# Audio-WestlakeU/FN-SSL

Measured on AMD Instinct MI355X. Metric: TF-frames/sec DP-IPD forward, 4-mic 257-bin x 300-frame, higher is better.
Workload: dtype f32; 1 GPU; BASELINE configs[1]: FN-SSL (online) DP-IPD forward, waveform->STFT->features->3x(full-band BiLSTM + narrow-band LSTM)->head; 32 utterances/GPU x 4 mics ('MM' = 6 pairs) x 257 bins x 300 frames, fp32; frame = one STFT frame of one utterance; stream_chunk_frames=0, utterances_per_gpu=32, global_batch=32, mics=4, pairs_per_utterance=6, frames=300, bins=257, parallelism=dp1 (utterance shards, no collective), chunk_pairs=0

## Files before the change

### fn-ssl_amd/csrc/lstm_f32c.h

```cpp
#pragma once

#include "lstm_static.h"

namespace fnssl_lstm {

constexpr int kF32cWaves = 16;

struct F32ClusterParams {
  unsigned* tags;
  unsigned* status;
  int clusters_per_dir;
  int groups_per_cluster;
  unsigned spin_limit;
  int stall_member;
  int rotate;
  int prio_mode;
};

template <int HH, int NV0, int NS0, int MODE, bool ABLRT = false, int DRIFT = 2, int NW_ = kF32cWaves, int GS = 1>
__global__ void __launch_bounds__(NW_ * 64) lstm_f32c_kernel(const LstmParams p, const F32ClusterParams cp) {
  constexpr int H = HH, NS = H / 16, NW = NW_;
  constexpr int NWS = NW / GS;
  static_assert((GS == 1 || GS == 4) && NW % GS == 0 && (NWS & (NWS - 1)) == 0, "gate split: whole slots, a power of two of them");
  constexpr bool SUM = (MODE & kSum) != 0, SAVE = (MODE & kSave) != 0;
  constexpr bool CAT = (MODE & kHas2) != 0;
  constexpr int QPS = 1 + NV0 + NS0 + NS;
  constexpr int XD = NW_ > 12 ? 4 : 8;
  constexpr bool STRH = H == 256 && GS == 1 && NW_ > 8;
  static_assert((CAT ? NS0 == 1 : !(NV0 && NS0)) && (NV0 == 0 || NV0 % XD == 0) && (H == 128 || H == 256),
                "blocks of src0, or its remainder alone, or blocks of src0 + the remainder quad of src2");
  static_assert(H == 128 || NW_ <= 8 || STRH, "H = 256 with the row of h_{t-1} held: at most two waves per SIMD (register budget)");
  static_assert(!STRH || (NV0 >= XD && (NV0 + NS) % XD == 0), "streamed row: the ring depth divides the block count");
  static_assert(GS == 1 || (!SAVE && !ABLRT), "gate split: inference kernels only");
  extern __shared__ __attribute__((aligned(16))) char smem[];
  const int ABL = ABLRT ? p.ablate : 0;

  const int b = blockIdx.x;
  const int m = (b >> 3) % NS;
  const int cl = ((b >> 3) / NS) * 8 + (b & 7);
  if (cl >= cp.clusters_per_dir * p.ndir) return;
  const int dir = cl / cp.clusters_per_dir;
  const int ck = cl - dir * cp.clusters_per_dir;
  const int g0 = ck * cp.groups_per_cluster;
  const int g1 = g0 + cp.groups_per_cluster < p.ntasks ? g0 + cp.groups_per_cluster : p.ntasks;
  if (__hip_atomic_load(cp.status, __ATOMIC_RELAXED, __HIP_MEMORY_SCOPE_AGENT) != 0) return;
  if (cl == 0 && m == cp.stall_member) return;

  const int lane = threadIdx.x & 63;
  const int n = lane & 15, g = lane >> 4;
  const int w = __builtin_amdgcn_readfirstlane((int)(threadIdx.x >> 6));
  const int ws = GS == 1 ? w : (w >> 2);
  const int gate = GS == 1 ? 0 : (w & 3);
  const bool rev = dir == 1;
  const unsigned vlane = lane * 16;

  {
    const v4f* src = reinterpret_cast<const v4f*>(reinterpret_cast<const char*>(p.wpack[dir]) + (size_t)(m * QPS) * 4096);
    v4f* dst = reinterpret_cast<v4f*>(smem);
    for (int i = threadIdx.x; i < QPS * 4 * 64; i += NW * 64) dst[i] = src[i];
  }
  char* const xch = smem + QPS * 4096;
  unsigned* const xcnt = reinterpret_cast<unsigned*>(xch + NWS * 2 * 4 * 1024);
  if (GS > 1 && threadIdx.x < NWS) xcnt[threadIdx.x] = 0;
  __syncthreads();
  const char* const lds_rd = smem + lane * 16;
  auto rec = [&](int q, int j) { return *reinterpret_cast<const v4f*>(lds_rd + (q * 4 + j) * 1024); };
  auto rec1 = [&](int q, int j) { return *reinterpret_cast<const float*>(lds_rd + (q * 4 + j) * 1024 + 4 * gate); };

  const unsigned st0 = (unsigned)(p.src0.st * 4), sto = (unsigned)(p.out_st * 4), stk = SUM ? (unsigned)(p.skip.st * 4) : 0u;
  const unsigned st2 = CAT ? (unsigned)(p.src2.st * 4) : 0u;
  const unsigned cy = (unsigned)p.carry;
  unsigned* const tag_cl = cp.tags + (size_t)cl * cp.groups_per_cluster * NS;
  const v4f zero4 = v4f{0.f, 0.f, 0.f, 0.f};

  unsigned pub_val = 0;
  unsigned* pub_tag = nullptr;
  auto pub_flush = [&]() {
    if (pub_tag) {
      asm volatile("s_waitcnt vmcnt(0)" ::: "memory");
      if (lane == 0) __hip_atomic_store(pub_tag, pub_val, __ATOMIC_RELAXED, __HIP_MEMORY_SCOPE_AGENT);
      pub_tag = nullptr;
    }
  };

  struct Grp {
    unsigned vo0, voo, vok, voo2, vo2 = 0;
    bool valid;
    int task, step;
  };
  auto locate = [&](int task, int qo0, int qi0, Grp& gr, rsrc_t& rx0, rsrc_t& ro, rsrc_t& rsk, rsrc_t& ro2, rsrc_t& rx2) {
    const int q0 = task * 16;
    gr.valid = q0 + n < p.nseq;
    const int d = q0 + n < p.nseq ? n : p.nseq - 1 - q0;
    const bool crossed = qi0 + d >= p.q_inner;
    auto one = [&](const float* base, long long so, long long si, int extra, unsigned& voff) {
      const long long delta = (long long)d * si + (crossed ? so - (long long)p.q_inner * si : 0ll);
      voff = (unsigned)(delta * 4) + (unsigned)(extra * 4);
      return make_rsrc(base + ((long long)qo0 * so + (long long)qi0 * si));
    };
    rx0 = one(p.src0.p, p.src0.so, p.src0.si, (NS0 && !CAT) ? g : 4 * g, gr.vo0);
    if constexpr (CAT) rx2 = one(p.src2.p, p.src2.so, p.src2.si, g, gr.vo2);
    ro = one(p.out, p.out_so, p.out_si, dir * H + 4 * g, gr.voo);
    gr.vok = gr.voo2 = 0;
    rsk = SUM ? one(p.skip.p, p.skip.so, p.skip.si, dir * H + 4 * g, gr.vok) : rx0;
    ro2 = SUM ? one(p.out_sum, p.out_so, p.out_si, dir * H + 4 * g, gr.voo2) : ro;
// ... 3 lines not shown
    return make_rsrc(cell_record<NS>(p.cscratch, p.ntasks, dir, task));
  };

  if (g0 + ws >= g1) return;
  unsigned long long clk0 = 0, rt0 = 0;
  if (ABLRT && (ABL & 512)) {
    clk0 = __builtin_amdgcn_s_memtime();
    rt0 = __builtin_amdgcn_s_memrealtime();
  }
  bool dead = false;
  auto bounded_wait = [&](auto ready, auto reload, int sleep, unsigned code) {
    for (unsigned spins = 0; !ready(); ++spins) {
      if (GS > 1) __builtin_amdgcn_s_sleep(1); else if (sleep == 8) __builtin_amdgcn_s_sleep(8); else __builtin_amdgcn_s_sleep(16);
      reload();
      const bool out = spins > cp.spin_limit;
      if (out || (spins & 63) == 63) {
        if (out) {
          if (lane == 0) __hip_atomic_store(cp.status, code | (unsigned)(cl & 0xffff), __ATOMIC_RELAXED, __HIP_MEMORY_SCOPE_AGENT);
          return false;
        }
        if (__hip_atomic_load(cp.status, __ATOMIC_RELAXED, __HIP_MEMORY_SCOPE_AGENT) != 0) return false;
      }
    }
    return true;
  };
  const int NGR = g1 - g0;
  const bool rot = cp.rotate && NGR >= 2 * NWS;
  const int FULL = rot ? (NGR / NWS) * NWS : NGR, LEFT = NGR - FULL;
  const bool single = GS == 1 && g0 + ws + NWS >= g1;
  Grp cur, nxt;
  rsrc_t rx0, ro, rsk, ro2, rx2, nrx0, nro, nrsk, nro2, nrx2;
  v4f xr[XD];
  float xs0 = 0.f;
  v4f cprev = zero4, skipv = zero4;
  unsigned tagv = 0, tagd = 0;
  auto request = [&](const Grp& gr, rsrc_t qx0, rsrc_t qsk, bool with_c, bool with_x = true) {
    const unsigned tt = tt_of(gr.step);
    if (!(ABL & 8)) {
      if constexpr (NV0 > 0) if (with_x) static_for<XD>([&](auto v) { xr[v.value] = bld4(qx0, gr.vo0, tt * st0 + 64 * v.value); });
      if constexpr (NS0 > 0 && !CAT) xs0 = bld1(qx0, gr.vo0, tt * st0);
    }
    if (SUM && !(ABL & 64)) skipv = bld4(qsk, gr.vok, tt * stk + 64 * m);
    if (gr.step > 0 || cy) {
      if (gr.step > 0 && !(ABL & 256))
        tagv = __hip_atomic_load(tag_cl + (size_t)(gr.task - g0) * NS + (lane & (NS - 1)), __ATOMIC_RELAXED, __HIP_MEMORY_SCOPE_AGENT);
      if (GS == 1 && with_c && !(ABL & 64)) cprev = bld4_l2(rc_of(gr.task), vlane, m * 1024);
    }
    if (DRIFT > 0 && !(ABL & 256) && gr.task - DRIFT * NWS >= g0)
      tagd = __hip_atomic_load(tag_cl + (size_t)(gr.task - DRIFT * NWS - g0) * NS + (lane & (NS - 1)), __ATOMIC_RELAXED, __HIP_MEMORY_SCOPE_AGENT);
  };
  cur.task = g0 + ws;
  cur.step = 0;
  unsigned iter = 0;
  const int qo_first = (cur.task * 16) / p.q_inner, qi_first = cur.task * 16 - qo_first * p.q_inner;
  int qo0 = qo_first, qi0 = qi_first;
  locate(cur.task, qo0, qi0, cur, rx0, ro, rsk, ro2, rx2);
  request(cur, rx0, rsk, true);
  if constexpr (CAT) xs0 = bld1(rx2, cur.vo2, tt_of(0) * st2);

  for (;;) {
    const int step = cur.step, task = cur.task;
    const unsigned tt = tt_of(step);
    const unsigned o0 = tt * st0, oo = (tt + cy) * sto;
    const unsigned op = (rev ? tt + 1 : tt - 1 + cy) * sto;
    const rsrc_t rc = rc_of(task);
    unsigned* const tag_g = tag_cl + (size_t)(task - g0) * NS;
    if (single && (step > 0 || cy) && !(ABL & 64)) cprev = bld4_l2(rc, vlane, m * 1024);
    const bool late_c = GS > 1 || task >= g0 + FULL;
    v4f cprev_cur = (step > 0 || cy) ? cprev : zero4;
    const v4f skip_cur = skipv;

    v4f hold[STRH ? 1 : NS];
    auto fetch_h = [&]() {
      if (DRIFT > 0 && !(ABL & 4) && !dead && task - DRIFT * NWS >= g0) {
        unsigned* const tag_d = tag_cl + (size_t)(task - DRIFT * NWS - g0) * NS;
        dead = !bounded_wait([&]() { return __builtin_amdgcn_ballot_w64(tagd < (unsigned)step + 1) == 0; },
                             [&]() { tagd = __hip_atomic_load(tag_d + (lane & (NS - 1)), __ATOMIC_RELAXED, __HIP_MEMORY_SCOPE_AGENT); }, 8, 0x40000u);
      }
      if ((step > 0 || cy) && !(ABL & 16)) {
        if (step > 0 && !(ABL & 4) && !dead)
          dead = !bounded_wait([&]() { return __builtin_amdgcn_ballot_w64(tagv < (unsigned)step) == 0; },
                               [&]() { tagv = __hip_atomic_load(tag_g + (lane & (NS - 1)), __ATOMIC_RELAXED, __HIP_MEMORY_SCOPE_AGENT); }, 16, 0x30000u);
        if (late_c && !(ABL & 64)) cprev_cur = bld4_l2(rc, vlane, m * 1024);
        if constexpr (!STRH) {
#pragma unroll
          for (int s = 0; s < NS; ++s) hold[s] = bld4_l2(ro, cur.voo, op + 64 * s);
        }
      } else if constexpr (!STRH) {
#pragma unroll
        for (int s = 0; s < NS; ++s) hold[s] = (ABL & 16) ? cprev : zero4;
      }
    };
    const bool hrow = step > 0 || cy;
    auto hblock = [&](int j) { return hrow ? bld4_l2(ro, cur.voo, op + 64 * j) : zero4; };

    if (cp.prio_mode == 2) __builtin_amdgcn_s_setprio(2);
    v4f acc[4];
    v4f ra[4];
    v4f acc1 = zero4;
    float rb[4] = {0.f, 0.f, 0.f, 0.f};
    if constexpr (GS == 1) {
      acc[0] = rec(0, 0);
      acc[1] = rec(0, 1);
      acc[2] = rec(0, 2);
      acc[3] = rec(0, 3);
      static_for<4>([&](auto j) { ra[j.value] = rec(1, j.value); });
    } else {
      acc1 = rec(0, gate);
      static_for<4>([&](auto j) { rb[j.value] = rec1(1, j.value); });
    }
    auto quad = [&](auto qc, float b0, float b1, float b2, float b3) {
      constexpr int Q = decltype(qc)::value;
      if constexpr (GS > 1) {
        acc1 = __builtin_amdgcn_mfma_f32_16x16x4f32(rb[0], b0, acc1, 0, 0, 0);
        if constexpr (Q + 1 < QPS) rb[0] = rec1(Q + 1, 0);
        acc1 = __builtin_amdgcn_mfma_f32_16x16x4f32(rb[1], b1, acc1, 0, 0, 0);
        if constexpr (Q + 1 < QPS) rb[1] = rec1(Q + 1, 1);
        acc1 = __builtin_amdgcn_mfma_f32_16x16x4f32(rb[2], b2, acc1, 0, 0, 0);
        if constexpr (Q + 1 < QPS) rb[2] = rec1(Q + 1, 2);
        acc1 = __builtin_amdgcn_mfma_f32_16x16x4f32(rb[3], b3, acc1, 0, 0, 0);
        if constexpr (Q + 1 < QPS) rb[3] = rec1(Q + 1, 3);
        return;
      }
      MFMA4(acc, ra[0], b0);
      __builtin_amdgcn_sched_barrier(0);
      if constexpr (Q + 1 < QPS) if (!(ABL & 128)) ra[0] = rec(Q + 1, 0);
      __builtin_amdgcn_sched_barrier(0);
      MFMA4(acc, ra[1], b1);
      __builtin_amdgcn_sched_barrier(0);
      if constexpr (Q + 1 < QPS) if (!(ABL & 128)) ra[1] = rec(Q + 1, 1);
      __builtin_amdgcn_sched_barrier(0);
      MFMA4(acc, ra[2], b2);
      __builtin_amdgcn_sched_barrier(0);
      if constexpr (Q + 1 < QPS) if (!(ABL & 128)) ra[2] = rec(Q + 1, 2);
      __builtin_amdgcn_sched_barrier(0);
      MFMA4(acc, ra[3], b3);
      __builtin_amdgcn_sched_barrier(0);
      if constexpr (Q + 1 < QPS) if (!(ABL & 128)) ra[3] = rec(Q + 1, 3);
      __builtin_amdgcn_sched_barrier(0);
    };
    auto quad1 = [&](auto qc, float b0) {
      constexpr int Q = decltype(qc)::value;
      if constexpr (GS > 1) {
        acc1 = __builtin_amdgcn_mfma_f32_16x16x4f32(rb[0], b0, acc1, 0, 0, 0);
        if constexpr (Q + 1 < QPS) static_for<4>([&](auto j) { rb[j.value] = rec1(Q + 1, j.value); });
        return;
      }
      MFMA4(acc, ra[0], b0);
      if constexpr (Q + 1 < QPS) static_for<4>([&](auto j) { ra[j.value] = rec(Q + 1, j.value); });
    };
    if constexpr (NV0 > 0) {
      static_for<NV0>([&](auto v) {
        constexpr int V = decltype(v)::value;
        if constexpr (STRH) {
          if constexpr (V == NV0 / 2) pub_flush();
          if constexpr (V == NV0 - XD) fetch_h();
        } else if constexpr (V == NV0 / 2) {
          pub_flush();
          fetch_h();
        }
        const v4f xb = xr[V % XD];
        quad(ic<1 + V>{}, xb.x, xb.y, xb.z, xb.w);
        if constexpr (V + XD < NV0) {
          if (!(ABL & 8)) xr[V % XD] = bld4(rx0, cur.vo0, o0 + 64 * (V + XD));
        } else if constexpr (STRH) {
          xr[V % XD] = hblock(V + XD - NV0);
        }
      });
      if constexpr (NS0 > 0) quad1(ic<1 + NV0>{}, xs0);
    } else {
      pub_flush();
      fetch_h();
      quad1(ic<1>{}, xs0);
    }
    bool seq_next = false;
    if (task < g0 + FULL && task + NWS < g0 + FULL) {
      nxt.task = task + NWS;
      nxt.step = step;
      seq_next = true;
    } else {
      const int j = (ws - step) & (NWS - 1);
      if (task < g0 + FULL && j < LEFT) {
// ... 20 lines not shown
            qi0 -= p.q_inner;
            ++qo0;
          }
        } else if (nxt.step == step) {
          qo0 = (nxt.task * 16) / p.q_inner;
          qi0 = nxt.task * 16 - qo0 * p.q_inner;
        } else {
          qo0 = qo_first;
          qi0 = qi_first;
        }
        locate(nxt.task, qo0, qi0, nxt, nrx0, nro, nrsk, nro2, nrx2);
      }
      request(nxt, nrx0, nrsk, !single && nxt.task < g0 + FULL, !STRH);
      if constexpr (CAT) xs0 = bld1(nrx2, nxt.vo2, tt_of(nxt.step) * st2);
    }
    static_for<NS>([&](auto sp) {
      constexpr int SP = decltype(sp)::value;
      if constexpr (STRH) {
        constexpr int B = NV0 + SP, B2 = B + XD;
        const v4f hb = xr[B % XD];
        quad(ic<1 + NV0 + NS0 + SP>{}, hb.x, hb.y, hb.z, hb.w);
        if constexpr (B2 < NV0 + NS) {
          xr[B % XD] = hblock(B2 - NV0);
        } else {
          if (more) xr[B % XD] = bld4(nrx0, nxt.vo0, tt_of(nxt.step) * st0 + 64 * (B2 - NV0 - NS));
        }
      } else {
        quad(ic<1 + NV0 + NS0 + SP>{}, hold[SP].x, hold[SP].y, hold[SP].z, hold[SP].w);
      }
    });

    if (cp.prio_mode == 2) __builtin_amdgcn_s_setprio(0);
    if (dead) break;
    v4f cn, hn;
    if (ABL & 2) {
      cn = acc[1] + cprev_cur + acc[0];
      hn = acc[3] + acc[2];
    } else {
      v4f ig, fg, gg, og;
      if constexpr (GS == 1) {
        ig = sigmoid4(acc[0]);
        fg = sigmoid4(acc[1]);
        gg = tanh4(acc[2]);
        og = sigmoid4(acc[3]);
      } else {
        const v4f act = gate == 2 ? tanh4(acc1) : sigmoid4(acc1);
        v4f* const xb = reinterpret_cast<v4f*>(xch + (size_t)((ws * 2 + (int)(iter & 1u)) * 4) * 1024);
        xb[gate * 64 + lane] = act;
        asm volatile("s_waitcnt lgkmcnt(0)" ::: "memory");
        if (lane == 0) __hip_atomic_fetch_add(xcnt + ws, 1u, __ATOMIC_RELAXED, __HIP_MEMORY_SCOPE_WORKGROUP);
        const unsigned want = 4u * (iter + 1u);
        for (unsigned spins = 0;; ++spins) {
          if (__hip_atomic_load(xcnt + ws, __ATOMIC_RELAXED, __HIP_MEMORY_SCOPE_WORKGROUP) >= want) break;
          if (dead || ((spins & 63u) == 63u && __hip_atomic_load(cp.status, __ATOMIC_RELAXED, __HIP_MEMORY_SCOPE_AGENT) != 0u) ||
              spins > cp.spin_limit) {
            dead = true;
            break;
          }
          __builtin_amdgcn_s_sleep(1);
        }
        asm volatile("" ::: "memory");
        ig = xb[lane];
        fg = xb[64 + lane];
        gg = xb[128 + lane];
        og = xb[192 + lane];
        ++iter;
      }
      cn = cell4(fg, cprev_cur, ig, gg);
      hn = mul_rn4(og, tanh4(cn));
      if constexpr (SAVE) {
        const rsrc_t rres = make_rsrc(reinterpret_cast<const char*>(p.reserve) +
                                      ((size_t)dir * p.ntasks + task) * p.nsteps * (size_t)(NS * kReserveRecs * 1024));
        const unsigned rb = (tt * NS + m) * (kReserveRecs * 1024);
        bst4(ig, rres, vlane, rb);
        bst4(fg, rres, vlane, rb + 1024);
        bst4(gg, rres, vlane, rb + 2048);
        bst4(og, rres, vlane, rb + 3072);
        bst4(cn, rres, vlane, rb + 4096);
      }
    }
    asm("" : "+v"(hn.x), "+v"(hn.y), "+v"(hn.z), "+v"(hn.w));
    if (ABL & 32) asm volatile("" ::"v"(cn), "v"(hn));
    const bool storer = GS == 1 || gate == 0;
    if (storer && !(ABL & 32)) bst4(cn, rc, vlane, m * 1024);
    if (storer && cur.valid && !(ABL & 32)) {
      __builtin_amdgcn_raw_buffer_store_b128(__builtin_bit_cast(v4u, hn), ro, cur.voo, oo + 64 * m, 16);
      if (SUM) bst4(add_rn4(hn, skip_cur), ro2, cur.voo2, oo + 64 * m);
    }
    pub_val = __builtin_amdgcn_readfirstlane((unsigned)step + 1);
    pub_tag = ((ABL & 256) || !storer) ? nullptr : tag_g + m;
    if (GS > 1 || single) pub_flush();
    if (!more || dead) break;
    cur = nxt;
    rx0 = nrx0;
    ro = nro;
    rsk = nrsk;
    ro2 = nro2;
    if constexpr (CAT) rx2 = nrx2;
  }
  pub_flush();
  asm volatile("s_waitcnt vmcnt(0)" ::: "memory");
  if (ABLRT && (ABL & 512) && (w == 0 || w == 15) && lane == 0) {
    const unsigned long long c1 = __builtin_amdgcn_s_memtime(), r1 = __builtin_amdgcn_s_memrealtime();
    printf("f32c blk %d wave %d start %llu end %llu cycles %llu MHz %.1f\n", b, w, rt0, r1, c1 - clk0,
           (double)(c1 - clk0) / (double)(r1 - rt0) * 100.0);
  }
}

template <int HH, int NV0, int NS0, int MODE, bool ABLRT = false, int DRIFT = 2, int NW_ = kF32cWaves, int GS = 1>
int launch_f32c_k(const LstmParams& p, const F32ClusterParams& cp, hipStream_t st) {
  constexpr int NS = HH / 16;
  constexpr int QPS = 1 + NV0 + NS0 + NS;
  const size_t lds = (size_t)QPS * 4096 + (GS > 1 ? (size_t)(NW_ / GS) * 8192 + 64 : 0);
  static_assert(QPS * 4096 + (GS > 1 ? (NW_ / GS) * 8192 + 64 : 0) <= 160 * 1024, "LDS");
  auto k = lstm_f32c_kernel<HH, NV0, NS0, MODE, ABLRT, DRIFT, NW_, GS>;
  if (lds > 48 * 1024)
    FNSSL_HIP(hipFuncSetAttribute(reinterpret_cast<const void*>(k), hipFuncAttributeMaxDynamicSharedMemorySize, (int)lds));
  const int ncl = cp.clusters_per_dir * p.ndir;
  const int nwg = 8 * NS * ((ncl + 7) / 8);
  if (!cluster_grid_fits(reinterpret_cast<const void*>(k), NW_ * 64, lds, nwg)) return kNoCluster;
  if (p.dry) return FNSSL_OK;
  hipLaunchKernelGGL(k, dim3(nwg), dim3(NW_ * 64), lds, st, p, cp);
  FNSSL_CHECK_LAUNCH("lstm_f32c_kernel");
  return FNSSL_OK;
}

}
```

### fn-ssl_amd/csrc/lstm_f32c.hip

```cpp
#include <cstdlib>

#include "lstm_f32c.h"
#include "tuning.h"

namespace fnssl_lstm {

constexpr int kF32cWavesH256 = 16;
constexpr int kF32cWavesH256Split = 8;

static bool f32c_uniform(const LstmParams& p, int mode) {
  auto even = [&](long long so, long long si) { return si >= 0 && so == (long long)p.q_inner * si; };
  return even(p.src0.so, p.src0.si) && even(p.out_so, p.out_si) && (!(mode & kSum) || even(p.skip.so, p.skip.si)) &&
         (!(mode & kHas2) || even(p.src2.so, p.src2.si));
}

bool f32c_handles(const LstmParams& p, int H, int mode) {
  if (fnssl::tune(FNSSL_TUNE_NO_F32_CLUSTER)) return false;
  if ((H != 128 && H != 256) || p.ablate) return false;
  if (H == 128) {
    if (p.c2 != 0 || p.carry) return false;
    if (p.reserve && mode != 0) return false;
    if (!(p.c0 == 256 && (mode == kSum || mode == 0)) && !(p.c0 == 4 && mode == 0 && !fnssl::tune(FNSSL_TUNE_NO_F32C_B1))) return false;
  } else {
    if (p.ndir != 1 || p.c0 != 256 || fnssl::tune(FNSSL_TUNE_NO_F32_SMALL)) return false;
    const bool plain = p.c2 == 0 && (mode == 0 || mode == kSum), cat = p.c2 == 4 && (mode == kHas2 || mode == (kHas2 | kSum));
    if (!plain && !cat) return false;
    if (p.reserve && ((mode & kSum) || p.carry)) return false;
  }
  auto grows = [&](long long so, long long si) { return si >= 0 && so >= (long long)(p.q_inner - 1) * si; };
  if (!f32c_uniform(p, mode) &&
      (p.q_inner < 16 || !grows(p.src0.so, p.src0.si) || !grows(p.out_so, p.out_si) ||
       ((mode & kSum) && !grows(p.skip.so, p.skip.si)) || ((mode & kHas2) && !grows(p.src2.so, p.src2.si))))
    return false;
  const int ncu = cluster_cus();
  if (ncu < (H / 16) * p.ndir) return false;
  const long long groups = (long long)p.ntasks * p.ndir;
  if (const int mg = fnssl::tune(FNSSL_TUNE_F32C_MIN_GROUPS, 1, 1 << 30)) {
    if (groups < mg) return false;
  }
  if (p.reserve) {
    if (fnssl::tune(FNSSL_TUNE_TRAIN_NO_F32_CLUSTER)) return false;
    return true;
  }
  if (H == 256) {
    const long long full = 12LL * ncu, rounds = (groups + full - 1) / full;
    return groups < full || groups * 100 < rounds * full * 97;
  }
  return !fnssl::tune(FNSSL_TUNE_NO_F32_SMALL) || groups >= 12LL * ncu;
}

int forward_f32c(LstmParams p, int H, int mode, size_t cluster_bytes, hipStream_t st) {
  if (f32c_uniform(p, mode)) p.q_inner = p.nseq;
  const int ncu = cluster_cus();
  const int members = H / 16;
  F32ClusterParams cp;
  cp.clusters_per_dir = (ncu / members) / p.ndir;
  cp.groups_per_cluster = (p.ntasks + cp.clusters_per_dir - 1) / cp.clusters_per_dir;
  cp.status = reinterpret_cast<unsigned*>(p.cluster_ws);
  cp.tags = reinterpret_cast<unsigned*>(p.cluster_ws + 256);
  cp.spin_limit = cluster_spin_limit();
  cp.stall_member = cluster_test_stall();
  cp.rotate = !fnssl::tune(FNSSL_TUNE_F32C_NO_ROTATE);
  cp.prio_mode = fnssl::tune(FNSSL_TUNE_F32C_PRIO, 9, 9) ? 0 : 2;
  const size_t tag_bytes = (size_t)p.ndir * cp.clusters_per_dir * cp.groups_per_cluster * members * sizeof(unsigned);
  FNSSL_REQUIRE(256 + tag_bytes <= cluster_bytes, "lstm_forward: the cluster kernel's tags exceed the workspace's cluster area");
  if (!p.dry) FNSSL_HIP(hipMemsetAsync(p.cluster_ws, 0, 256 + tag_bytes, st));
  const int gs_knob = fnssl::tune(FNSSL_TUNE_F32C_GATE_SPLIT, 1, 4);
  const bool gsplit = gs_knob ? gs_knob == 4 : cp.groups_per_cluster <= 1;
  if (H == 256) {
    constexpr int W = kF32cWavesH256;
    if (p.reserve)
      return p.c2 == 4 ? launch_f32c_k<256, 16, 1, kHas2 | kSave, false, 2, W>(p, cp, st) : launch_f32c_k<256, 16, 0, kSave, false, 2, W>(p, cp, st);
    if (gsplit) {
      if (mode == (kHas2 | kSum)) return launch_f32c_k<256, 16, 1, kHas2 | kSum, false, 2, kF32cWavesH256Split, 4>(p, cp, st);
      if (mode == kHas2) return launch_f32c_k<256, 16, 1, kHas2, false, 2, kF32cWavesH256Split, 4>(p, cp, st);
      if (mode == kSum) return launch_f32c_k<256, 16, 0, kSum, false, 2, kF32cWavesH256Split, 4>(p, cp, st);
      return launch_f32c_k<256, 16, 0, 0, false, 2, kF32cWavesH256Split, 4>(p, cp, st);
    }
    if (cp.groups_per_cluster <= kF32cWavesH256Split) {
      constexpr int W8 = kF32cWavesH256Split;
      if (mode == (kHas2 | kSum)) return launch_f32c_k<256, 16, 1, kHas2 | kSum, false, 2, W8>(p, cp, st);
      if (mode == kHas2) return launch_f32c_k<256, 16, 1, kHas2, false, 2, W8>(p, cp, st);
      if (mode == kSum) return launch_f32c_k<256, 16, 0, kSum, false, 2, W8>(p, cp, st);
      return launch_f32c_k<256, 16, 0, 0, false, 2, W8>(p, cp, st);
    }
    if (mode == (kHas2 | kSum)) return launch_f32c_k<256, 16, 1, kHas2 | kSum, false, 2, W>(p, cp, st);
    if (mode == kHas2) return launch_f32c_k<256, 16, 1, kHas2, false, 2, W>(p, cp, st);
    if (mode == kSum) return launch_f32c_k<256, 16, 0, kSum, false, 2, W>(p, cp, st);
    return launch_f32c_k<256, 16, 0, 0, false, 2, W>(p, cp, st);
  }
  if (gsplit && !p.reserve) {
    if (p.c0 == 4) return launch_f32c_k<128, 0, 1, 0, false, 2, kF32cWaves, 4>(p, cp, st);
    if (mode == kSum) return launch_f32c_k<128, 16, 0, kSum, false, 2, kF32cWaves, 4>(p, cp, st);
    return launch_f32c_k<128, 16, 0, 0, false, 2, kF32cWaves, 4>(p, cp, st);
  }
#ifdef FNSSL_BUILD_ABLATE
  if (const int abl = env_int("FNSSL_F32C_ABL", 1, 1023)) {
    p.ablate = abl;
    if (mode == kSum) return launch_f32c_k<128, 16, 0, kSum, true>(p, cp, st);
// ... 12 lines not shown
```

### fn-ssl_amd/csrc/runtime.hip

```cpp
#include <atomic>
#include <cstring>
#include <map>
#include <mutex>
#include <string>
#include <vector>

#include "common.h"
#include "tuning.h"

namespace fnssl {

int device_cus() {
  static std::mutex mu;
  static int cache[64] = {0};
  int dev = 0;
  if (hipGetDevice(&dev) != hipSuccess || dev < 0 || dev >= 64) return 256;
  std::lock_guard<std::mutex> lk(mu);
  if (cache[dev] == 0) {
    int n = 0;
    if (hipDeviceGetAttribute(&n, hipDeviceAttributeMultiprocessorCount, dev) != hipSuccess || n <= 0) n = 256;
    cache[dev] = n;
  }
  return cache[dev];
}
// ... 20 lines not shown
    "LSTM_CHQ",
    "NO_F32_CLUSTER",
    "NO_F32C_B1",
    "TRAIN_NO_F32_CLUSTER",
    "F32C_NO_ROTATE",
    "F32C_PRIO",
    "NO_CLUSTER",
    "NO_CLUSTER_B1",
    "NO_CLUSTER_H128",
    "CLUSTER_SPREAD",
    "BF16P_DRAIN",
    "BF16W_SOLO",
    "BWD_NO_CLUSTER",
    "BWD_CLUSTER_MIN_GROUPS",
    "BWD_CLUSTER_NO_ROTATE",
    "BWDC_NO_PREFETCH",
    "BWDC_NO_TOKEN",
    "BWDC_WAVES16",
    "FWD_RING",
    "BWD_RING",
    "TRAIN_SPLIT",
    "TRAIN_NO_STATIC",
    "NO_FWD2",
    "NO_BWD2",
    "SN_SCALAR",
    "STFT_PER_FRAME",
    "CLUSTER_SPIN_LIMIT",
    "CLUSTER_TEST_STALL",
    "RESERVED_CUS",
    "NO_F32_SMALL",
    "F32C_MIN_GROUPS",
    "F32C_GATE_SPLIT",
    "CLUSTER_FULL_TILES",
    "NO_STATIC4"};
constexpr int kTuneNamed = (int)(sizeof(kTuneNames) / sizeof(kTuneNames[0]));
static_assert(kTuneNamed <= FNSSL_TUNE_COUNT, "more knob names than slots");
static_assert(kTuneNamed == FNSSL_TUNE_NO_STATIC4 + 1, "knob names out of step with include/fnssl.h");
}

const fnssl_tuning& tuning() {
  if (g_call_tuning) return *g_call_tuning;
  const unsigned v = g_tuning_version.load(std::memory_order_acquire);
  if (v != g_thread_version) {
    std::lock_guard<std::mutex> lk(g_tuning_mu);
    g_thread_tuning = g_default_tuning;
    g_thread_version = g_tuning_version.load(std::memory_order_relaxed);
  }
  return g_thread_tuning;
}

TuningScope::TuningScope(const fnssl_tuning* t) : prev_(g_call_tuning), active_(false) {
  if (t && t->struct_bytes == sizeof(fnssl_tuning)) {
    g_call_tuning = t;
    active_ = true;
  }
}
TuningScope::~TuningScope() {
  if (active_) g_call_tuning = prev_;
}

void set_error(const char* fmt, ...) {
  va_list ap;
  va_start(ap, fmt);
  vsnprintf(g_err, sizeof(g_err), fmt, ap);
  va_end(ap);
}

namespace {
struct Rec {
  const char* name;
// ... 191 lines not shown
```

### fn-ssl_amd/fnssl/_lib.py

```python
from __future__ import annotations

import ctypes as C
import os

import torch

_HERE = os.path.dirname(os.path.abspath(__file__))
LIB_PATH = os.path.join(os.path.dirname(_HERE), "csrc", "libfnssl_hip.so")
LIB_PATH = os.environ.get("FNSSL_LIB_PATH", LIB_PATH)

ABI_VERSION = 19
CH_MODE = {"M": 0, "MM": 1}
LSTM_FAMILY = {1: "generic", 2: "static", 3: "static2 (retired)", 4: "split", 5: "split_static", 6: "f32_cluster",
               7: "static3", 8: "bf16", 9: "bf16_solo", 10: "bf16_pair", 11: "bf16_cluster", 12: "train", 13: "bwd", 14: "bwd_cluster",
               15: "static4"}

SYMBOLS = [
    "fnssl_abi_version", "fnssl_last_error", "fnssl_tuning_set", "fnssl_tuning_get", "fnssl_tuning_name", "fnssl_occupy_cus", "fnssl_num_frames", "fnssl_num_pairs", "fnssl_stft",
    "fnssl_num_frames_ex", "fnssl_stft_ex", "fnssl_array_frontend",
    "fnssl_forgetting_coefs", "fnssl_pair_features", "fnssl_nchw_to_seq", "fnssl_lstm_packed_floats",
    "fnssl_lstm_pack", "fnssl_lstm_workspace_bytes", "fnssl_lstm_workspace_bytes_ex", "fnssl_lstm_plan_rounds", "fnssl_lstm_plan", "fnssl_lstm_forward", "fnssl_lstm_cluster_status", "fnssl_head", "fnssl_linear",
    "fnssl_ipd2doa", "fnssl_doa_peaks", "fnssl_dpipd_targets", "fnssl_conv3x3_packed_floats", "fnssl_conv3x3_pack", "fnssl_conv3x3_causal",
    "fnssl_avgpool_time", "fnssl_array_features", "fnssl_conv3x3_packed_floats_bf16", "fnssl_conv3x3_pack_bf16",
    "fnssl_conv3x3_causal_bf16", "fnssl_conv3x3_causal_bf16a",
# ... 239 lines not shown
    lib.fnssl_train_map_bytes.restype = sz
    lib.fnssl_train_upload_maps.argtypes = [vp, vp, vp]
    lib.fnssl_train_workspace_bytes.argtypes = [vp, i, i, i]
    lib.fnssl_train_workspace_bytes.restype = sz
    lib.fnssl_train_backward.argtypes = [vp, vp, vp, vp, vp, i, i, i, i, C.c_uint, ll, ll, vp, vp, sz, vp]
    lib.fnssl_train_step.argtypes = [vp, vp, vp, vp, vp, vp, vp, i, i, i, i, C.c_uint, f, f, f, f, i, vp, vp, sz, vp]
    PV = C.POINTER(BtfView)
    lib.fnssl_sn_layernorm.argtypes = [vp, ll, i, vp, vp, f, vp, vp]
    lib.fnssl_sn_encoder.argtypes = [vp, ll, ll, ll, ll, i, i, i, i, vp, vp, vp, vp, vp, ll, ll, ll, i, vp]
    lib.fnssl_sn_fconv.argtypes = [PV, i, i, i, C.POINTER(SnFconvW), i, i, vp, ll, ll, ll, i, vp]
    lib.fnssl_sn_full.argtypes = [PV, i, i, i, C.POINTER(SnFullW), i, vp, ll, ll, ll, i, vp]
    lib.fnssl_sn_mamba_workspace_bytes.argtypes = [i, i, i]
    lib.fnssl_sn_mamba_workspace_bytes.restype = sz
    lib.fnssl_sn_mamba.argtypes = [PV, i, i, i, C.POINTER(SnMambaW), i, i, vp, vp, i, vp, ll, ll, ll, vp, sz, i, vp]
    lib.fnssl_sn_head.argtypes = [PV, i, i, i, vp, vp, vp, vp, vp, vp]
    lib.fnssl_sn_forward_workspace_bytes.argtypes = [i, i, i]
    lib.fnssl_sn_forward_workspace_bytes.restype = sz
    lib.fnssl_sn_state_floats.argtypes = [C.POINTER(SnNet), i, i]
    lib.fnssl_sn_state_floats.restype = sz
    lib.fnssl_sn_forward.argtypes = [C.POINTER(SnNet), vp, ll, ll, ll, ll, i, i, i, vp, i, vp, vp, sz, vp]
    lib.fnssl_timing_enable.argtypes = [i]
    lib.fnssl_timing_select.argtypes = [C.c_char_p]
    lib.fnssl_timing_collect.argtypes = [i, vp, vp, vp, vp]
    if lib.fnssl_abi_version() != ABI_VERSION:
        raise RuntimeError("fnssl: ABI version mismatch (library %d, binding %d)"
                           % (lib.fnssl_abi_version(), ABI_VERSION))
    _lib = lib
    refresh_tuning()
    return lib


_tune_index = None
_PRESENCE = {"NO_F32_CLUSTER", "NO_F32C_B1", "TRAIN_NO_F32_CLUSTER", "F32C_NO_ROTATE", "NO_CLUSTER", "NO_CLUSTER_B1",
             "NO_CLUSTER_H128", "CLUSTER_SPREAD", "BF16W_SOLO", "SN_SCALAR", "STFT_PER_FRAME"}
_ENV_ALIAS = {"LSTM_NO_STATIC": "FNSSL_LSTM_NO_STATIC"}


def tuning_names():
    global _tune_index
    if _tune_index is None:
        lib = _lib
        if lib is None:
            raise RuntimeError("fnssl: load() first")
        idx, k = {}, 0
        while True:
            n = lib.fnssl_tuning_name(k)
            if n is None:
                break
            idx[n.decode()] = k
            k += 1
        _tune_index = idx
    return _tune_index


def tuning_from_env(environ=None) -> Tuning:
    environ = os.environ if environ is None else environ
    t = Tuning()
    t.struct_bytes = C.sizeof(Tuning)
    for name, k in tuning_names().items():
        v = environ.get(_ENV_ALIAS.get(name, "FNSSL_" + name))
        if v is None:
            continue
        try:
            iv = int(v)
        except ValueError:
            iv = 1
        if name in _PRESENCE:
# ... 54 lines not shown
```

### include/fnssl.h

```cpp
#ifndef FNSSL_H_
#define FNSSL_H_

#include <stddef.h>

#ifdef __cplusplus
extern "C" {
#endif

#define FNSSL_ABI_VERSION 19

#define FNSSL_OK 0
#define FNSSL_E_INVALID (-1)
#define FNSSL_E_HIP (-2)
#define FNSSL_E_WORKSPACE (-3)

#define FNSSL_CH_MODE_M 0
#define FNSSL_CH_MODE_MM 1

#define FNSSL_WIN_LEN 512
#define FNSSL_HOP 256
#define FNSSL_NBIN 257
#define FNSSL_NF 256
#define FNSSL_SEG_FRAMES 12

// ... 13 lines not shown
#define FNSSL_TUNE_NO_F32_CLUSTER 9
#define FNSSL_TUNE_NO_F32C_B1 10
#define FNSSL_TUNE_TRAIN_NO_F32_CLUSTER 11
#define FNSSL_TUNE_F32C_NO_ROTATE 12
#define FNSSL_TUNE_F32C_PRIO 13
#define FNSSL_TUNE_NO_CLUSTER 14
#define FNSSL_TUNE_NO_CLUSTER_B1 15
#define FNSSL_TUNE_NO_CLUSTER_H128 16
#define FNSSL_TUNE_CLUSTER_SPREAD 17
#define FNSSL_TUNE_BF16P_DRAIN 18
#define FNSSL_TUNE_BF16W_SOLO 19
#define FNSSL_TUNE_BWD_NO_CLUSTER 20
#define FNSSL_TUNE_BWD_CLUSTER_MIN_GROUPS 21
#define FNSSL_TUNE_BWD_CLUSTER_NO_ROTATE 22
#define FNSSL_TUNE_BWDC_NO_PREFETCH 23
#define FNSSL_TUNE_BWDC_NO_TOKEN 24
#define FNSSL_TUNE_BWDC_WAVES16 25
#define FNSSL_TUNE_FWD_RING 26
#define FNSSL_TUNE_BWD_RING 27
#define FNSSL_TUNE_TRAIN_SPLIT 28
#define FNSSL_TUNE_TRAIN_NO_STATIC 29
#define FNSSL_TUNE_NO_FWD2 30
#define FNSSL_TUNE_NO_BWD2 31
#define FNSSL_TUNE_SN_SCALAR 32
#define FNSSL_TUNE_STFT_PER_FRAME 33
#define FNSSL_TUNE_CLUSTER_SPIN_LIMIT 34
#define FNSSL_TUNE_CLUSTER_TEST_STALL 35
#define FNSSL_TUNE_RESERVED_CUS 36
#define FNSSL_TUNE_NO_F32_SMALL 37
#define FNSSL_TUNE_F32C_MIN_GROUPS 38
#define FNSSL_TUNE_F32C_GATE_SPLIT 39
#define FNSSL_TUNE_CLUSTER_FULL_TILES 40
#define FNSSL_TUNE_NO_STATIC4 41
#define FNSSL_TUNE_COUNT 48

typedef struct fnssl_tuning {
  unsigned struct_bytes;
  int knob[FNSSL_TUNE_COUNT];
} fnssl_tuning;

int fnssl_tuning_set(const fnssl_tuning* t);
int fnssl_tuning_get(fnssl_tuning* t);
const char* fnssl_tuning_name(int index);

int fnssl_occupy_cus(int nblocks, int lds_bytes, unsigned* stop, int max_ms, void* stream);


int fnssl_num_frames(int ns);

int fnssl_num_pairs(int nch, int ch_mode);

int fnssl_stft(const float* sig, int nb, int ns, int nch,
               long long sb, long long sn, long long sc,
               float* spec, float* magsum, void* stream);

int fnssl_num_frames_ex(int ns, int hop, int center);
int fnssl_stft_ex(const float* sig, int nb, int ns, int nch,
                  long long sb, long long sn, long long sc, int hop, int center,
                  float* spec, float* magsum, void* stream);

int fnssl_forgetting_coefs(int nt, int sample_length, float* a, float* b);

int fnssl_pair_features(const float* spec, const float* magsum,
                        const float* coef_a, const float* coef_b,
                        int nb, int nch, int nt, int ch_mode, float eps,
                        float* mu, float* x, int layout, void* stream);
// ... 362 lines not shown
```

Baseline: 17690 frames/s.

## Give each f32 cluster member two hidden slices for block 1 full-band layer

Adds an SPM template parameter so that each cluster workgroup owns two 16-wide hidden slices instead of one. For the H=128 full-band inference layer (c0==4, no reserve), the cluster shrinks from 8 members to 4, which doubles the number of clusters and spreads recurrent groups over more clusters when enough groups exist. Each member now holds twice the weight records in LDS and runs interleaved MFMA chains for both slices. In exchange, per-step work per member doubles and LDS and register use rise, while cross-member tag synchronisation per step drops. A new tuning knob can disable the path.

Result: no change. 17770 frames/s, median of 6 (+0.5%).

```diff
diff --git a/fn-ssl_amd/csrc/lstm_f32c.h b/fn-ssl_amd/csrc/lstm_f32c.h
--- a/fn-ssl_amd/csrc/lstm_f32c.h
+++ b/fn-ssl_amd/csrc/lstm_f32c.h
@@ -17,9 +17,12 @@
   int prio_mode;
 };
 
-template <int HH, int NV0, int NS0, int MODE, bool ABLRT = false, int DRIFT = 2, int NW_ = kF32cWaves, int GS = 1>
+template <int HH, int NV0, int NS0, int MODE, bool ABLRT = false, int DRIFT = 2, int NW_ = kF32cWaves, int GS = 1, int SPM = 1>
 __global__ void __launch_bounds__(NW_ * 64) lstm_f32c_kernel(const LstmParams p, const F32ClusterParams cp) {
   constexpr int H = HH, NS = H / 16, NW = NW_;
+  constexpr int NM = NS / SPM;
+  static_assert(SPM == 1 || (SPM == 2 && H == 128 && NV0 == 0 && NS0 == 1 && MODE == 0 && GS == 1 && !ABLRT),
+                "two slices per member: block 1's full-band inference layer only");
   constexpr int NWS = NW / GS;
   static_assert((GS == 1 || GS == 4) && NW % GS == 0 && (NWS & (NWS - 1)) == 0, "gate split: whole slots, a power of two of them");
   constexpr bool SUM = (MODE & kSum) != 0, SAVE = (MODE & kSave) != 0;
@@ -36,8 +39,8 @@
   const int ABL = ABLRT ? p.ablate : 0;
 
   const int b = blockIdx.x;
-  const int m = (b >> 3) % NS;
-  const int cl = ((b >> 3) / NS) * 8 + (b & 7);
+  const int m = (b >> 3) % NM;
+  const int cl = ((b >> 3) / NM) * 8 + (b & 7);
   if (cl >= cp.clusters_per_dir * p.ndir) return;
   const int dir = cl / cp.clusters_per_dir;
   const int ck = cl - dir * cp.clusters_per_dir;
@@ -55,22 +58,24 @@
   const unsigned vlane = lane * 16;
 
   {
-    const v4f* src = reinterpret_cast<const v4f*>(reinterpret_cast<const char*>(p.wpack[dir]) + (size_t)(m * QPS) * 4096);
+    const v4f* src = reinterpret_cast<const v4f*>(reinterpret_cast<const char*>(p.wpack[dir]) + (size_t)(m * SPM * QPS) * 4096);
     v4f* dst = reinterpret_cast<v4f*>(smem);
-    for (int i = threadIdx.x; i < QPS * 4 * 64; i += NW * 64) dst[i] = src[i];
+    for (int i = threadIdx.x; i < SPM * QPS * 4 * 64; i += NW * 64) dst[i] = src[i];
   }
-  char* const xch = smem + QPS * 4096;
+  char* const xch = smem + SPM * QPS * 4096;
   unsigned* const xcnt = reinterpret_cast<unsigned*>(xch + NWS * 2 * 4 * 1024);
   if (GS > 1 && threadIdx.x < NWS) xcnt[threadIdx.x] = 0;
   __syncthreads();
   const char* const lds_rd = smem + lane * 16;
-  auto rec = [&](int q, int j) { return *reinterpret_cast<const v4f*>(lds_rd + (q * 4 + j) * 1024); };
+  auto recs = [&](int k, int q, int j) { return *reinterpret_cast<const v4f*>(lds_rd + ((k * QPS + q) * 4 + j) * 1024); };
+  auto rec = [&](int q, int j) { return recs(0, q, j); };
   auto rec1 = [&](int q, int j) { return *reinterpret_cast<const float*>(lds_rd + (q * 4 + j) * 1024 + 4 * gate); };
 
   const unsigned st0 = (unsigned)(p.src0.st * 4), sto = (unsigned)(p.out_st * 4), stk = SUM ? (unsigned)(p.skip.st * 4) : 0u;
   const unsigned st2 = CAT ? (unsigned)(p.src2.st * 4) : 0u;
   const unsigned cy = (unsigned)p.carry;
-  unsigned* const tag_cl = cp.tags + (size_t)cl * cp.groups_per_cluster * NS;
+  unsigned* const tag_cl = cp.tags + (size_t)cl * cp.groups_per_cluster * NM;
+  const int s0 = m * SPM;
   const v4f zero4 = v4f{0.f, 0.f, 0.f, 0.f};
 
   unsigned pub_val = 0;
@@ -140,7 +145,8 @@
   rsrc_t rx0, ro, rsk, ro2, rx2, nrx0, nro, nrsk, nro2, nrx2;
   v4f xr[XD];
   float xs0 = 0.f;
-  v4f cprev = zero4, skipv = zero4;
+  v4f cprev[SPM], skipv = zero4;
+  static_for<SPM>([&](auto k) { cprev[k.value] = zero4; });
   unsigned tagv = 0, tagd = 0;
   auto request = [&](const Grp& gr, rsrc_t qx0, rsrc_t qsk, bool with_c, bool with_x = true) {
     const unsigned tt = tt_of(gr.step);
@@ -148,14 +154,15 @@
       if constexpr (NV0 > 0) if (with_x) static_for<XD>([&](auto v) { xr[v.value] = bld4(qx0, gr.vo0, tt * st0 + 64 * v.value); });
       if constexpr (NS0 > 0 && !CAT) xs0 = bld1(qx0, gr.vo0, tt * st0);
     }
-    if (SUM && !(ABL & 64)) skipv = bld4(qsk, gr.vok, tt * stk + 64 * m);
+    if (SUM && !(ABL & 64)) skipv = bld4(qsk, gr.vok, tt * stk + 64 * s0);
     if (gr.step > 0 || cy) {
       if (gr.step > 0 && !(ABL & 256))
-        tagv = __hip_atomic_load(tag_cl + (size_t)(gr.task - g0) * NS + (lane & (NS - 1)), __ATOMIC_RELAXED, __HIP_MEMORY_SCOPE_AGENT);
-      if (GS == 1 && with_c && !(ABL & 64)) cprev = bld4_l2(rc_of(gr.task), vlane, m * 1024);
+        tagv = __hip_atomic_load(tag_cl + (size_t)(gr.task - g0) * NM + (lane & (NM - 1)), __ATOMIC_RELAXED, __HIP_MEMORY_SCOPE_AGENT);
+      if (GS == 1 && with_c && !(ABL & 64))
+        static_for<SPM>([&](auto k) { cprev[k.value] = bld4_l2(rc_of(gr.task), vlane, (s0 + k.value) * 1024); });
     }
     if (DRIFT > 0 && !(ABL & 256) && gr.task - DRIFT * NWS >= g0)
-      tagd = __hip_atomic_load(tag_cl + (size_t)(gr.task - DRIFT * NWS - g0) * NS + (lane & (NS - 1)), __ATOMIC_RELAXED, __HIP_MEMORY_SCOPE_AGENT);
+      tagd = __hip_atomic_load(tag_cl + (size_t)(gr.task - DRIFT * NWS - g0) * NM + (lane & (NM - 1)), __ATOMIC_RELAXED, __HIP_MEMORY_SCOPE_AGENT);
   };
   cur.task = g0 + ws;
   cur.step = 0;
@@ -172,47 +179,47 @@
     const unsigned o0 = tt * st0, oo = (tt + cy) * sto;
     const unsigned op = (rev ? tt + 1 : tt - 1 + cy) * sto;
     const rsrc_t rc = rc_of(task);
-    unsigned* const tag_g = tag_cl + (size_t)(task - g0) * NS;
-    if (single && (step > 0 || cy) && !(ABL & 64)) cprev = bld4_l2(rc, vlane, m * 1024);
+    unsigned* const tag_g = tag_cl + (size_t)(task - g0) * NM;
+    if (single && (step > 0 || cy) && !(ABL & 64))
+      static_for<SPM>([&](auto k) { cprev[k.value] = bld4_l2(rc, vlane, (s0 + k.value) * 1024); });
     const bool late_c = GS > 1 || task >= g0 + FULL;
-    v4f cprev_cur = (step > 0 || cy) ? cprev : zero4;
+    v4f cprev_cur[SPM];
+    static_for<SPM>([&](auto k) { cprev_cur[k.value] = (step > 0 || cy) ? cprev[k.value] : zero4; });
     const v4f skip_cur = skipv;
 
     v4f hold[STRH ? 1 : NS];
     auto fetch_h = [&]() {
       if (DRIFT > 0 && !(ABL & 4) && !dead && task - DRIFT * NWS >= g0) {
-        unsigned* const tag_d = tag_cl + (size_t)(task - DRIFT * NWS - g0) * NS;
+        unsigned* const tag_d = tag_cl + (size_t)(task - DRIFT * NWS - g0) * NM;
         dead = !bounded_wait([&]() { return __builtin_amdgcn_ballot_w64(tagd < (unsigned)step + 1) == 0; },
-                             [&]() { tagd = __hip_atomic_load(tag_d + (lane & (NS - 1)), __ATOMIC_RELAXED, __HIP_MEMORY_SCOPE_AGENT); }, 8, 0x40000u);
+                             [&]() { tagd = __hip_atomic_load(tag_d + (lane & (NM - 1)), __ATOMIC_RELAXED, __HIP_MEMORY_SCOPE_AGENT); }, 8, 0x40000u);
       }
       if ((step > 0 || cy) && !(ABL & 16)) {
         if (step > 0 && !(ABL & 4) && !dead)
           dead = !bounded_wait([&]() { return __builtin_amdgcn_ballot_w64(tagv < (unsigned)step) == 0; },
-                               [&]() { tagv = __hip_atomic_load(tag_g + (lane & (NS - 1)), __ATOMIC_RELAXED, __HIP_MEMORY_SCOPE_AGENT); }, 16, 0x30000u);
-        if (late_c && !(ABL & 64)) cprev_cur = bld4_l2(rc, vlane, m * 1024);
+                               [&]() { tagv = __hip_atomic_load(tag_g + (lane & (NM - 1)), __ATOMIC_RELAXED, __HIP_MEMORY_SCOPE_AGENT); }, 16, 0x30000u);
+        if (late_c && !(ABL & 64))
+          static_for<SPM>([&](auto k) { cprev_cur[k.value] = bld4_l2(rc, vlane, (s0 + k.value) * 1024); });
         if constexpr (!STRH) {
 #pragma unroll
           for (int s = 0; s < NS; ++s) hold[s] = bld4_l2(ro, cur.voo, op + 64 * s);
         }
       } else if constexpr (!STRH) {
 #pragma unroll
-        for (int s = 0; s < NS; ++s) hold[s] = (ABL & 16) ? cprev : zero4;
+        for (int s = 0; s < NS; ++s) hold[s] = (ABL & 16) ? cprev[0] : zero4;
       }
     };
     const bool hrow = step > 0 || cy;
     auto hblock = [&](int j) { return hrow ? bld4_l2(ro, cur.voo, op + 64 * j) : zero4; };
 
     if (cp.prio_mode == 2) __builtin_amdgcn_s_setprio(2);
-    v4f acc[4];
+    v4f acc[SPM][4];
     v4f ra[4];
     v4f acc1 = zero4;
     float rb[4] = {0.f, 0.f, 0.f, 0.f};
     if constexpr (GS == 1) {
-      acc[0] = rec(0, 0);
-      acc[1] = rec(0, 1);
-      acc[2] = rec(0, 2);
-      acc[3] = rec(0, 3);
-      static_for<4>([&](auto j) { ra[j.value] = rec(1, j.value); });
+      static_for<SPM>([&](auto k) { static_for<4>([&](auto j) { acc[k.value][j.value] = recs(k.value, 0, j.value); }); });
+      static_for<4>([&](auto r) { ra[r.value] = recs(r.value % SPM, 1, r.value / SPM); });
     } else {
       acc1 = rec(0, gate);
       static_for<4>([&](auto j) { rb[j.value] = rec1(1, j.value); });
@@ -230,22 +237,15 @@
         if constexpr (Q + 1 < QPS) rb[3] = rec1(Q + 1, 3);
         return;
       }
-      MFMA4(acc, ra[0], b0);
-      __builtin_amdgcn_sched_barrier(0);
-      if constexpr (Q + 1 < QPS) if (!(ABL & 128)) ra[0] = rec(Q + 1, 0);
-      __builtin_amdgcn_sched_barrier(0);
-      MFMA4(acc, ra[1], b1);
-      __builtin_amdgcn_sched_barrier(0);
-      if constexpr (Q + 1 < QPS) if (!(ABL & 128)) ra[1] = rec(Q + 1, 1);
-      __builtin_amdgcn_sched_barrier(0);
-      MFMA4(acc, ra[2], b2);
-      __builtin_amdgcn_sched_barrier(0);
-      if constexpr (Q + 1 < QPS) if (!(ABL & 128)) ra[2] = rec(Q + 1, 2);
-      __builtin_amdgcn_sched_barrier(0);
-      MFMA4(acc, ra[3], b3);
-      __builtin_amdgcn_sched_barrier(0);
-      if constexpr (Q + 1 < QPS) if (!(ABL & 128)) ra[3] = rec(Q + 1, 3);
-      __builtin_amdgcn_sched_barrier(0);
+      const float bq[4] = {b0, b1, b2, b3};
+      static_for<4 * SPM>([&](auto rc) {
+        constexpr int R = decltype(rc)::value, J = R / SPM, K = R % SPM;
+        constexpr int N = R + 4, QN = Q + N / (4 * SPM), JN = N % (4 * SPM) / SPM, KN = N % SPM;
+        MFMA4(acc[K], ra[R % 4], bq[J]);
+        __builtin_amdgcn_sched_barrier(0);
+        if constexpr (QN < QPS) if (!(ABL & 128)) ra[R % 4] = recs(KN, QN, JN);
+        __builtin_amdgcn_sched_barrier(0);
+      });
     };
     auto quad1 = [&](auto qc, float b0) {
       constexpr int Q = decltype(qc)::value;
@@ -254,8 +254,8 @@
         if constexpr (Q + 1 < QPS) static_for<4>([&](auto j) { rb[j.value] = rec1(Q + 1, j.value); });
         return;
       }
-      MFMA4(acc, ra[0], b0);
-      if constexpr (Q + 1 < QPS) static_for<4>([&](auto j) { ra[j.value] = rec(Q + 1, j.value); });
+      static_for<SPM>([&](auto k) { MFMA4(acc[k.value], ra[k.value], b0); });
+      if constexpr (Q + 1 < QPS) static_for<4>([&](auto r) { ra[r.value] = recs(r.value % SPM, Q + 1, r.value / SPM); });
     };
     if constexpr (NV0 > 0) {
       static_for<NV0>([&](auto v) {
@@ -342,61 +342,65 @@
 
     if (cp.prio_mode == 2) __builtin_amdgcn_s_setprio(0);
     if (dead) break;
-    v4f cn, hn;
-    if (ABL & 2) {
-      cn = acc[1] + cprev_cur + acc[0];
-      hn = acc[3] + acc[2];
-    } else {
-      v4f ig, fg, gg, og;
-      if constexpr (GS == 1) {
-        ig = sigmoid4(acc[0]);
-        fg = sigmoid4(acc[1]);
-        gg = tanh4(acc[2]);
-        og = sigmoid4(acc[3]);
+    const bool storer = GS == 1 || gate == 0;
+    static_for<SPM>([&](auto kc) {
+      constexpr int K = decltype(kc)::value;
+      const int sl = s0 + K;
+      v4f cn, hn;
+      if (ABL & 2) {
+        cn = acc[K][1] + cprev_cur[K] + acc[K][0];
+        hn = acc[K][3] + acc[K][2];
       } else {
-        const v4f act = gate == 2 ? tanh4(acc1) : sigmoid4(acc1);
-        v4f* const xb = reinterpret_cast<v4f*>(xch + (size_t)((ws * 2 + (int)(iter & 1u)) * 4) * 1024);
-        xb[gate * 64 + lane] = act;
-        asm volatile("s_waitcnt lgkmcnt(0)" ::: "memory");
-        if (lane == 0) __hip_atomic_fetch_add(xcnt + ws, 1u, __ATOMIC_RELAXED, __HIP_MEMORY_SCOPE_WORKGROUP);
-        const unsigned want = 4u * (iter + 1u);
-        for (unsigned spins = 0;; ++spins) {
-          if (__hip_atomic_load(xcnt + ws, __ATOMIC_RELAXED, __HIP_MEMORY_SCOPE_WORKGROUP) >= want) break;
-          if (dead || ((spins & 63u) == 63u && __hip_atomic_load(cp.status, __ATOMIC_RELAXED, __HIP_MEMORY_SCOPE_AGENT) != 0u) ||
-              spins > cp.spin_limit) {
-            dead = true;
-            break;
+        v4f ig, fg, gg, og;
+        if constexpr (GS == 1) {
+          ig = sigmoid4(acc[K][0]);
+          fg = sigmoid4(acc[K][1]);
+          gg = tanh4(acc[K][2]);
+          og = sigmoid4(acc[K][3]);
+        } else {
+          const v4f act = gate == 2 ? tanh4(acc1) : sigmoid4(acc1);
+          v4f* const xb = reinterpret_cast<v4f*>(xch + (size_t)((ws * 2 + (int)(iter & 1u)) * 4) * 1024);
+          xb[gate * 64 + lane] = act;
+          asm volatile("s_waitcnt lgkmcnt(0)" ::: "memory");
+          if (lane == 0) __hip_atomic_fetch_add(xcnt + ws, 1u, __ATOMIC_RELAXED, __HIP_MEMORY_SCOPE_WORKGROUP);
+          const unsigned want = 4u * (iter + 1u);
+          for (unsigned spins = 0;; ++spins) {
+            if (__hip_atomic_load(xcnt + ws, __ATOMIC_RELAXED, __HIP_MEMORY_SCOPE_WORKGROUP) >= want) break;
+            if (dead || ((spins & 63u) == 63u && __hip_atomic_load(cp.status, __ATOMIC_RELAXED, __HIP_MEMORY_SCOPE_AGENT) != 0u) ||
+                spins > cp.spin_limit) {
+              dead = true;
+              break;
+            }
+            __builtin_amdgcn_s_sleep(1);
           }
-          __builtin_amdgcn_s_sleep(1);
-        }
-        asm volatile("" ::: "memory");
-        ig = xb[lane];
-        fg = xb[64 + lane];
-        gg = xb[128 + lane];
-        og = xb[192 + lane];
-        ++iter;
-      }
-      cn = cell4(fg, cprev_cur, ig, gg);
-      hn = mul_rn4(og, tanh4(cn));
-      if constexpr (SAVE) {
-        const rsrc_t rres = make_rsrc(reinterpret_cast<const char*>(p.reserve) +
-                                      ((size_t)dir * p.ntasks + task) * p.nsteps * (size_t)(NS * kReserveRecs * 1024));
-        const unsigned rb = (tt * NS + m) * (kReserveRecs * 1024);
-        bst4(ig, rres, vlane, rb);
-        bst4(fg, rres, vlane, rb + 1024);
-        bst4(gg, rres, vlane, rb + 2048);
-        bst4(og, rres, vlane, rb + 3072);
-        bst4(cn, rres, vlane, rb + 4096);
-      }
-    }
-    asm("" : "+v"(hn.x), "+v"(hn.y), "+v"(hn.z), "+v"(hn.w));
-    if (ABL & 32) asm volatile("" ::"v"(cn), "v"(hn));
-    const bool storer = GS == 1 || gate == 0;
-    if (storer && !(ABL & 32)) bst4(cn, rc, vlane, m * 1024);
-    if (storer && cur.valid && !(ABL & 32)) {
-      __builtin_amdgcn_raw_buffer_store_b128(__builtin_bit_cast(v4u, hn), ro, cur.voo, oo + 64 * m, 16);
-      if (SUM) bst4(add_rn4(hn, skip_cur), ro2, cur.voo2, oo + 64 * m);
-    }
+          asm volatile("" ::: "memory");
+          ig = xb[lane];
+          fg = xb[64 + lane];
+          gg = xb[128 + lane];
+          og = xb[192 + lane];
+          ++iter;
+        }
+        cn = cell4(fg, cprev_cur[K], ig, gg);
+        hn = mul_rn4(og, tanh4(cn));
+        if constexpr (SAVE) {
+          const rsrc_t rres = make_rsrc(reinterpret_cast<const char*>(p.reserve) +
+                                        ((size_t)dir * p.ntasks + task) * p.nsteps * (size_t)(NS * kReserveRecs * 1024));
+          const unsigned rb = (tt * NS + sl) * (kReserveRecs * 1024);
+          bst4(ig, rres, vlane, rb);
+          bst4(fg, rres, vlane, rb + 1024);
+          bst4(gg, rres, vlane, rb + 2048);
+          bst4(og, rres, vlane, rb + 3072);
+          bst4(cn, rres, vlane, rb + 4096);
+        }
+      }
+      asm("" : "+v"(hn.x), "+v"(hn.y), "+v"(hn.z), "+v"(hn.w));
+      if (ABL & 32) asm volatile("" ::"v"(cn), "v"(hn));
+      if (storer && !(ABL & 32)) bst4(cn, rc, vlane, sl * 1024);
+      if (storer && cur.valid && !(ABL & 32)) {
+        __builtin_amdgcn_raw_buffer_store_b128(__builtin_bit_cast(v4u, hn), ro, cur.voo, oo + 64 * sl, 16);
+        if (SUM) bst4(add_rn4(hn, skip_cur), ro2, cur.voo2, oo + 64 * sl);
+      }
+    });
     pub_val = __builtin_amdgcn_readfirstlane((unsigned)step + 1);
     pub_tag = ((ABL & 256) || !storer) ? nullptr : tag_g + m;
     if (GS > 1 || single) pub_flush();
@@ -417,17 +421,17 @@
   }
 }
 
-template <int HH, int NV0, int NS0, int MODE, bool ABLRT = false, int DRIFT = 2, int NW_ = kF32cWaves, int GS = 1>
+template <int HH, int NV0, int NS0, int MODE, bool ABLRT = false, int DRIFT = 2, int NW_ = kF32cWaves, int GS = 1, int SPM = 1>
 int launch_f32c_k(const LstmParams& p, const F32ClusterParams& cp, hipStream_t st) {
-  constexpr int NS = HH / 16;
+  constexpr int NS = HH / 16, NM = NS / SPM;
   constexpr int QPS = 1 + NV0 + NS0 + NS;
-  const size_t lds = (size_t)QPS * 4096 + (GS > 1 ? (size_t)(NW_ / GS) * 8192 + 64 : 0);
-  static_assert(QPS * 4096 + (GS > 1 ? (NW_ / GS) * 8192 + 64 : 0) <= 160 * 1024, "LDS");
-  auto k = lstm_f32c_kernel<HH, NV0, NS0, MODE, ABLRT, DRIFT, NW_, GS>;
+  const size_t lds = (size_t)SPM * QPS * 4096 + (GS > 1 ? (size_t)(NW_ / GS) * 8192 + 64 : 0);
+  static_assert(SPM * QPS * 4096 + (GS > 1 ? (NW_ / GS) * 8192 + 64 : 0) <= 160 * 1024, "LDS");
+  auto k = lstm_f32c_kernel<HH, NV0, NS0, MODE, ABLRT, DRIFT, NW_, GS, SPM>;
   if (lds > 48 * 1024)
     FNSSL_HIP(hipFuncSetAttribute(reinterpret_cast<const void*>(k), hipFuncAttributeMaxDynamicSharedMemorySize, (int)lds));
   const int ncl = cp.clusters_per_dir * p.ndir;
-  const int nwg = 8 * NS * ((ncl + 7) / 8);
+  const int nwg = 8 * NM * ((ncl + 7) / 8);
   if (!cluster_grid_fits(reinterpret_cast<const void*>(k), NW_ * 64, lds, nwg)) return kNoCluster;
   if (p.dry) return FNSSL_OK;
   hipLaunchKernelGGL(k, dim3(nwg), dim3(NW_ * 64), lds, st, p, cp);
diff --git a/fn-ssl_amd/csrc/lstm_f32c.hip b/fn-ssl_amd/csrc/lstm_f32c.hip
--- a/fn-ssl_amd/csrc/lstm_f32c.hip
+++ b/fn-ssl_amd/csrc/lstm_f32c.hip
@@ -52,19 +52,36 @@
 int forward_f32c(LstmParams p, int H, int mode, size_t cluster_bytes, hipStream_t st) {
   if (f32c_uniform(p, mode)) p.q_inner = p.nseq;
   const int ncu = cluster_cus();
-  const int members = H / 16;
   F32ClusterParams cp;
-  cp.clusters_per_dir = (ncu / members) / p.ndir;
-  cp.groups_per_cluster = (p.ntasks + cp.clusters_per_dir - 1) / cp.clusters_per_dir;
+  auto geometry = [&](int members) {
+    cp.clusters_per_dir = (ncu / members) / p.ndir;
+    cp.groups_per_cluster = (p.ntasks + cp.clusters_per_dir - 1) / cp.clusters_per_dir;
+  };
+  geometry(H / 16);
+  bool two = false;
+#ifdef FNSSL_BUILD_ABLATE
+  const bool abl_on = env_int("FNSSL_F32C_ABL", 1, 1023) != 0;
+#else
+  constexpr bool abl_on = false;
+#endif
+  if (H == 128 && !abl_on && p.c0 == 4 && mode == 0 && !p.reserve && !fnssl::tune(FNSSL_TUNE_F32C_B1_ONE_SLICE) &&
+      !fnssl::tune(FNSSL_TUNE_F32C_GATE_SPLIT, 1, 4)) {
+    geometry(H / 32);
+    two = cp.groups_per_cluster >= 2 * kF32cWaves;
+    if (!two) geometry(H / 16);
+  }
+  const int members = two ? H / 32 : H / 16;
   cp.status = reinterpret_cast<unsigned*>(p.cluster_ws);
   cp.tags = reinterpret_cast<unsigned*>(p.cluster_ws + 256);
   cp.spin_limit = cluster_spin_limit();
   cp.stall_member = cluster_test_stall();
+  if (two && cp.stall_member >= 0) cp.stall_member /= 2;
   cp.rotate = !fnssl::tune(FNSSL_TUNE_F32C_NO_ROTATE);
   cp.prio_mode = fnssl::tune(FNSSL_TUNE_F32C_PRIO, 9, 9) ? 0 : 2;
   const size_t tag_bytes = (size_t)p.ndir * cp.clusters_per_dir * cp.groups_per_cluster * members * sizeof(unsigned);
   FNSSL_REQUIRE(256 + tag_bytes <= cluster_bytes, "lstm_forward: the cluster kernel's tags exceed the workspace's cluster area");
   if (!p.dry) FNSSL_HIP(hipMemsetAsync(p.cluster_ws, 0, 256 + tag_bytes, st));
+  if (two) return launch_f32c_k<128, 0, 1, 0, false, 2, kF32cWaves, 1, 2>(p, cp, st);
   const int gs_knob = fnssl::tune(FNSSL_TUNE_F32C_GATE_SPLIT, 1, 4);
   const bool gsplit = gs_knob ? gs_knob == 4 : cp.groups_per_cluster <= 1;
   if (H == 256) {
diff --git a/fn-ssl_amd/csrc/runtime.hip b/fn-ssl_amd/csrc/runtime.hip
--- a/fn-ssl_amd/csrc/runtime.hip
+++ b/fn-ssl_amd/csrc/runtime.hip
@@ -76,10 +76,11 @@
     "F32C_MIN_GROUPS",
     "F32C_GATE_SPLIT",
     "CLUSTER_FULL_TILES",
-    "NO_STATIC4"};
+    "NO_STATIC4",
+    "F32C_B1_ONE_SLICE"};
 constexpr int kTuneNamed = (int)(sizeof(kTuneNames) / sizeof(kTuneNames[0]));
 static_assert(kTuneNamed <= FNSSL_TUNE_COUNT, "more knob names than slots");
-static_assert(kTuneNamed == FNSSL_TUNE_NO_STATIC4 + 1, "knob names out of step with include/fnssl.h");
+static_assert(kTuneNamed == FNSSL_TUNE_F32C_B1_ONE_SLICE + 1, "knob names out of step with include/fnssl.h");
 }
 
 const fnssl_tuning& tuning() {
diff --git a/fn-ssl_amd/fnssl/_lib.py b/fn-ssl_amd/fnssl/_lib.py
--- a/fn-ssl_amd/fnssl/_lib.py
+++ b/fn-ssl_amd/fnssl/_lib.py
@@ -295,7 +295,7 @@
 
 _tune_index = None
 _PRESENCE = {"NO_F32_CLUSTER", "NO_F32C_B1", "TRAIN_NO_F32_CLUSTER", "F32C_NO_ROTATE", "NO_CLUSTER", "NO_CLUSTER_B1",
-             "NO_CLUSTER_H128", "CLUSTER_SPREAD", "BF16W_SOLO", "SN_SCALAR", "STFT_PER_FRAME"}
+             "NO_CLUSTER_H128", "CLUSTER_SPREAD", "BF16W_SOLO", "SN_SCALAR", "STFT_PER_FRAME", "F32C_B1_ONE_SLICE"}
 _ENV_ALIAS = {"LSTM_NO_STATIC": "FNSSL_LSTM_NO_STATIC"}
 
 
diff --git a/include/fnssl.h b/include/fnssl.h
--- a/include/fnssl.h
+++ b/include/fnssl.h
@@ -69,6 +69,7 @@
 #define FNSSL_TUNE_F32C_GATE_SPLIT 39
 #define FNSSL_TUNE_CLUSTER_FULL_TILES 40
 #define FNSSL_TUNE_NO_STATIC4 41
+#define FNSSL_TUNE_F32C_B1_ONE_SLICE 42
 #define FNSSL_TUNE_COUNT 48
 
 typedef struct fnssl_tuning {
```
